# KinWaiCheuk/ReconVAT

Measured on AMD Instinct MI355X. Metric: training audio-sec/sec (node), higher is better.
Workload: dtype f32; 1 GPU; ReconVAT UNet_Onset VAT=True reconstruction=True, per-GPU B_l=8 + B_ul=8 segments of 327680 samples (640 frames x 229 mel), Adam+StepLR, fp32; parallelism=dp1, hipgraph=True, two_stream_schedule=True, kernel_plan_table=644fe159bb9eb70e, kernel_plan_mode=table, vat_nan_flag=0

## Files before the change

### reconvat_amd/csrc/attn.hip

```cpp
#include "common.h"
#include <stdlib.h>
#include <mutex>

#ifndef RV_ATTN_ABL
#define RV_ATTN_ABL 0
#endif
#define AT_W 31
#define AT_P 15
#define AT_TT 16
#define AT_WIN (AT_TT + 2 * AT_P)
#define AT_WINP 48
#define AT_NW 5
#define AT_NTHR (AT_NW * 64)
#define AT_SLD 80
#define AT_A2LD 52
#define AT_A3LD 84
#define AT_MAXT 4

struct AttnArgs {
    const float* q; const float* k; const float* v; long ld;
    const float* rel;
    float* out; float* att;
    const float* dout; const float* de_in;
    float* dq; float* dk; float* dv; long dld;
    float* de;
    int B, L, G, dh, dhp;
    int v4, dv4;
    int seq_kv;
    int rel_regs;
};

__device__ __attribute__((aligned(16))) const float rv_attn_zero[256] = {0.f};

__device__ __forceinline__ int stage_rows(float* dst, int ldk, const float* src, long ld, int col0, int dh, int dhp,
                                          int row0, int nvalid, int ntotal, int L, bool v4) {
    int issued = 0;
    const int wave = __builtin_amdgcn_readfirstlane(threadIdx.x >> 6), lane = threadIdx.x & 63;
    const int per = v4 ? 256 : 64;
    const int nfull = v4 ? (dh & ~3) : dh;
    const int ninst = (nfull + per - 1) / per;
    const int rem = dh - nfull;
    const int lf = v4 ? lane * 4 : lane;
    const float* s = src + ((long)(row0 + wave) * ld + col0) + lf;
    const float* z = rv_attn_zero + lf;
    float* drow = dst + wave * ldk;
    const long sstep = (long)AT_NW * ld;
    const int dstep = AT_NW * ldk;
    const int npad = dhp - dh;
    for (int r = wave; r < ntotal; r += AT_NW, s += sstep, drow += dstep) {
        const int t = row0 + r;
        const bool real = r < nvalid && t >= 0 && t < L;
        if (v4) {
            for (int k = 0; k < ninst; ++k)
                if (k * 256 + lf < nfull) glds16(real ? s + k * 256 : z, drow + k * 256);
            if (rem) {
                if (lane < rem) glds4(real ? s - lf + nfull + lane : rv_attn_zero + lane, drow + nfull);
                ++issued;
            }
        } else {
            for (int k = 0; k < ninst; ++k)
                if (k * 64 + lf < dh) glds4(real ? s + k * 64 : z, drow + k * 64);
        }
        issued += ninst;
        if (lane < npad) drow[dh + lane] = 0.f;
    }
    return issued;
}
__device__ __forceinline__ void stage_wait() { asm volatile("s_waitcnt vmcnt(0)" ::: "memory"); }

__device__ __forceinline__ f32x4 score_tile(const float* X, const float* Y, int ldk, int nchunk, int i, int g4) {
    f32x4 acc = (f32x4){0.f, 0.f, 0.f, 0.f};
    const float* xp = X + i * ldk + 4 * g4;
    const float* yp = Y + i * ldk + 4 * g4;
    for (int c = 0; c < nchunk; ++c) {
        const f32x4 a4 = *reinterpret_cast<const f32x4*>(xp + 16 * c);
        const f32x4 b4 = *reinterpret_cast<const f32x4*>(yp + 16 * c);
#pragma unroll
        for (int r = 0; r < 4; ++r) acc = __builtin_amdgcn_mfma_f32_16x16x4f32(a4[r], b4[r], acc, 0, 0, 0);
    }
    return acc;
}

__device__ __forceinline__ f32x4 score_tile_regs(const float* X, const f32x4 (&yb)[16], int ldk, int nchunk, int i, int g4) {
    f32x4 acc = (f32x4){0.f, 0.f, 0.f, 0.f};
    const float* xp = X + i * ldk + 4 * g4;
#pragma unroll
    for (int c = 0; c < 16; ++c) {
        if (c < nchunk) {
            const f32x4 a4 = *reinterpret_cast<const f32x4*>(xp + 16 * c);
#pragma unroll
            for (int r = 0; r < 4; ++r) acc = __builtin_amdgcn_mfma_f32_16x16x4f32(a4[r], yb[c][r], acc, 0, 0, 0);
        }
    }
    return acc;
}

struct RelFrag { f32x4 y[AT_MAXT][2]; };
__device__ __forceinline__ void rel_frag_load(RelFrag& rf, const float* relT, int F, int col0, int dh, int ntiles) {
    const int lane = threadIdx.x & 63, wave = threadIdx.x >> 6;
    const int i = lane & 15, g4 = lane >> 4;
#pragma unroll
    for (int q = 0; q < AT_MAXT; ++q) {
        const int f = 16 * (wave + AT_NW * q) + i;
        const bool fok = wave + AT_NW * q < ntiles && f < dh;
#pragma unroll
        for (int c = 0; c < 2; ++c)
#pragma unroll
            for (int r = 0; r < 4; ++r) {
                const int w = 16 * c + 4 * g4 + r;
                rf.y[q][c][r] = (fok && w < AT_W) ? relT[(long)w * F + col0 + f] : 0.f;
            }
    }
}

template <int NCH>
__device__ __forceinline__ void apply_tiles(const float* A, int lda, const float* Y, int ldk, int ntiles, float* dst,
                                            long dld, int col0, int dh, int nrows_valid, const RelFrag* rf = nullptr) {
    const int lane = threadIdx.x & 63, wave = threadIdx.x >> 6;
    const int i = lane & 15, g4 = lane >> 4;
    f32x4 acc[AT_MAXT];
#pragma unroll
    for (int q = 0; q < AT_MAXT; ++q) acc[q] = (f32x4){0.f, 0.f, 0.f, 0.f};
    if (rf) {
#pragma unroll
        for (int c = 0; c < 2; ++c) {
            const f32x4 a4 = *reinterpret_cast<const f32x4*>(A + i * lda + 16 * (NCH + c) + 4 * g4);
#pragma unroll
            for (int q = 0; q < AT_MAXT; ++q) {
                if (wave + AT_NW * q < ntiles) {
#pragma unroll
                    for (int r = 0; r < 4; ++r) acc[q] = __builtin_amdgcn_mfma_f32_16x16x4f32(a4[r], rf->y[q][c][r], acc[q], 0, 0, 0);
                }
            }
        }
    }
#pragma unroll
    for (int c = 0; c < NCH; ++c) {
        const f32x4 a4 = *reinterpret_cast<const f32x4*>(A + i * lda + 16 * c + 4 * g4);
        const float* yk = Y + (16 * c + 4 * g4) * ldk + i;
#pragma unroll
        for (int q = 0; q < AT_MAXT; ++q) {
            const int nt = wave + AT_NW * q;
            if (nt < ntiles) {
#pragma unroll
                for (int r = 0; r < 4; ++r)
                    acc[q] = __builtin_amdgcn_mfma_f32_16x16x4f32(a4[r], yk[r * ldk + 16 * nt], acc[q], 0, 0, 0);
            }
        }
    }
#pragma unroll
    for (int q = 0; q < AT_MAXT; ++q) {
        const int nt = wave + AT_NW * q;
        const int f = 16 * nt + i;
        if (nt >= ntiles || f >= dh) continue;
#pragma unroll
        for (int r = 0; r < 4; ++r) {
            const int t = 4 * g4 + r;
            if (t < nrows_valid) dst[(long)t * dld + col0 + f] = acc[q][r];
        }
    }
}

__device__ __forceinline__ float grp16_sum(float v) {
#pragma unroll
    for (int o = 8; o > 0; o >>= 1) v += __shfl_xor(v, o, 64);
    return v;
}
__device__ __forceinline__ float grp16_max(float v) {
#pragma unroll
    for (int o = 8; o > 0; o >>= 1) v = fmaxf(v, __shfl_xor(v, o, 64));
    return v;
}

__global__ __launch_bounds__(AT_NTHR) void attn_fwd_k(AttnArgs a) {
    extern __shared__ __attribute__((aligned(16))) float smem[];
    const int dh = a.dh, dhp = a.dhp, ldk = dhp + 4, nchunk = dhp >> 4, F = a.G * dh;
    float* Qs = smem;
    float* Kx = Qs + AT_TT * ldk;
    float* Sr = Kx + (a.rel_regs ? AT_WINP : 80) * ldk;
    float* A2 = Sr + AT_TT * AT_SLD;
    const int ntile = (a.L + AT_TT - 1) / AT_TT;
    const int bx = xcd_remap(blockIdx.x, gridDim.x);
    const int b = bx / ntile, t0 = (bx - b * ntile) * AT_TT;
    const int g = blockIdx.y;
    const int tid = threadIdx.x, lane = tid & 63, wave = tid >> 6;
    const int i = lane & 15, g4 = lane >> 4;
    const long boff = (long)b * a.L * a.ld;
    if (RV_ATTN_ABL & 16) return;
    if (!(RV_ATTN_ABL & 1)) {
    stage_rows(Qs, ldk, a.q + boff, a.ld, g * dh, dh, dhp, t0, AT_TT, AT_TT, a.L, a.v4);
    stage_rows(Kx, ldk, a.k + boff, a.ld, g * dh, dh, dhp, t0 - AT_P, AT_WIN, AT_WINP, a.L, a.v4);
    }
    f32x4 yb[16];
    if (a.rel_regs) {
        if (wave >= 3) {
            const int w = 16 * (wave - 3) + i;
            const float* rp = a.rel + (long)min(w, AT_W - 1) * F + g * dh + 4 * g4;
#pragma unroll
            for (int c = 0; c < 16; ++c)
#pragma unroll
                for (int r = 0; r < 4; ++r) yb[c][r] = (c < nchunk && w < AT_W && 16 * c + 4 * g4 + r < dh) ? rp[16 * c + r] : 0.f;
        }
    } else if (!(RV_ATTN_ABL & 1)) {
        stage_rows(Kx + AT_WINP * ldk, ldk, a.rel, F, g * dh, dh, dhp, 0, AT_W, 32, AT_W, a.dv4);
    }
    for (int idx = tid; idx < AT_TT * AT_A2LD; idx += AT_NTHR) A2[idx] = 0.f;
    stage_wait();
    __syncthreads();
    if (!(RV_ATTN_ABL & 2)) {
        const f32x4 s = (a.rel_regs && wave >= 3) ? score_tile_regs(Qs, yb, ldk, nchunk, i, g4)
                                                  : score_tile(Qs, Kx + 16 * wave * ldk, ldk, nchunk, i, g4);
#pragma unroll
        for (int r = 0; r < 4; ++r) Sr[(4 * g4 + r) * AT_SLD + 16 * wave + i] = s[r];
    }
    __syncthreads();
    if (!(RV_ATTN_ABL & 1)) stage_rows(Kx, ldk, a.v + boff, a.ld, g * dh, dh, dhp, t0 - AT_P, AT_WIN, AT_WINP, a.L, a.v4);
    if (tid < 256 && !(RV_ATTN_ABL & 4)) {
        const int t = tid >> 4, l = tid & 15;
        const float* sr = Sr + t * AT_SLD;
        const float e0 = sr[t + l] + sr[AT_WINP + l];
        const float e1 = l < 15 ? sr[t + l + 16] + sr[AT_WINP + l + 16] : -INFINITY;
        const float m = grp16_max(fmaxf(e0, e1));
        float p0 = expf(e0 - m), p1 = l < 15 ? expf(e1 - m) : 0.f;
        const float inv = 1.f / grp16_sum(p0 + p1);
        p0 *= inv; p1 *= inv;
        A2[t * AT_A2LD + t + l] = p0;
        if (l < 15) A2[t * AT_A2LD + t + l + 16] = p1;
        if (a.att && t0 + t < a.L) {
            float* ar = a.att + (((long)b * a.L + t0 + t) * a.G + g) * AT_W;
            ar[l] = p0;
            if (l < 15) ar[l + 16] = p1;
        }
    }
    stage_wait();
    __syncthreads();
    if (!(RV_ATTN_ABL & 8)) apply_tiles<3>(A2, AT_A2LD, Kx, ldk, nchunk, a.out + ((long)b * a.L + t0) * F, F, g * dh, dh, a.L - t0);
}

__global__ __launch_bounds__(AT_NTHR) void attn_bwd_q_k(AttnArgs a) {
    extern __shared__ __attribute__((aligned(16))) float smem[];
    const int dh = a.dh, dhp = a.dhp, ldk = dhp + 4, nchunk = dhp >> 4, F = a.G * dh;
    float* Ds = smem;
    float* Kx = Ds + AT_TT * ldk;
    float* Sr = Kx + (a.rel_regs ? AT_WINP : 80) * ldk;
    float* A3 = Sr + AT_TT * AT_SLD;
    const int ntile = (a.L + AT_TT - 1) / AT_TT;
    const int bx = xcd_remap(blockIdx.x, gridDim.x);
    const int b = bx / ntile, t0 = (bx - b * ntile) * AT_TT;
    const int g = blockIdx.y;
    const int tid = threadIdx.x, lane = tid & 63, wave = tid >> 6;
    const int i = lane & 15, g4 = lane >> 4;
    const long boff = (long)b * a.L * a.ld;
    stage_rows(Ds, ldk, a.dout + (long)b * a.L * F, F, g * dh, dh, dhp, t0, AT_TT, AT_TT, a.L, a.dv4);
    stage_rows(Kx, ldk, a.v + boff, a.ld, g * dh, dh, dhp, t0 - AT_P, AT_WIN, AT_WINP, a.L, a.v4);
    RelFrag rf;
    if (a.rel_regs) rel_frag_load(rf, a.rel, F, g * dh, dh, nchunk);
    else stage_rows(Kx + AT_WINP * ldk, ldk, a.rel, F, g * dh, dh, dhp, 0, AT_W, 32, AT_W, a.dv4);
    for (int idx = tid; idx < AT_TT * AT_A3LD; idx += AT_NTHR) A3[idx] = 0.f;
    stage_wait();
    __syncthreads();
    if (wave < 3) {
        const f32x4 s = score_tile(Ds, Kx + 16 * wave * ldk, ldk, nchunk, i, g4);
#pragma unroll
        for (int r = 0; r < 4; ++r) Sr[(4 * g4 + r) * AT_SLD + 16 * wave + i] = s[r];
    }
    __syncthreads();
    stage_rows(Kx, ldk, a.k + boff, a.ld, g * dh, dh, dhp, t0 - AT_P, AT_WIN, AT_WINP, a.L, a.v4);
    if (tid < 256) {
        const int t = tid >> 4, l = tid & 15;
        const bool rv = t0 + t < a.L;
        const long arow = (((long)b * a.L + t0 + t) * a.G + g) * AT_W;
        const float p0 = rv ? a.att[arow + l] : 0.f;
        const float p1 = (rv && l < 15) ? a.att[arow + l + 16] : 0.f;
        const float* sr = Sr + t * AT_SLD;
        const float d0 = sr[t + l], d1 = l < 15 ? sr[t + l + 16] : 0.f;
        const float dot = grp16_sum(p0 * d0 + p1 * d1);
        const float e0 = p0 * (d0 - dot), e1 = p1 * (d1 - dot);
        float* ar = A3 + t * AT_A3LD;
        ar[t + l] = e0;
        ar[AT_WINP + l] = e0;
        if (l < 15) { ar[t + l + 16] = e1; ar[AT_WINP + l + 16] = e1; }
        if (rv) {
            a.de[arow + l] = e0;
            if (l < 15) a.de[arow + l + 16] = e1;
        }
    }
    stage_wait();
    __syncthreads();
    if (a.rel_regs) apply_tiles<3>(A3, AT_A3LD, Kx, ldk, nchunk, a.dq + ((long)b * a.L + t0) * a.dld, a.dld, g * dh, dh, a.L - t0, &rf);
    else apply_tiles<5>(A3, AT_A3LD, Kx, ldk, nchunk, a.dq + ((long)b * a.L + t0) * a.dld, a.dld, g * dh, dh, a.L - t0);
}

__global__ __launch_bounds__(AT_NTHR) void attn_bwd_kv_k(AttnArgs a) {
    extern __shared__ __attribute__((aligned(16))) float smem[];
    const int dh = a.dh, dhp = a.dhp, ldk = dhp + 4, nchunk = dhp >> 4, F = a.G * dh;
    float* Yd = smem;
    float* Yq = a.seq_kv ? Yd : Yd + AT_WINP * ldk;
    float* Ca = Yq + AT_WINP * ldk;
    float* Ce = Ca + AT_WINP * 32;
    float* A4 = Ce + AT_WINP * 32;
    float* A5 = A4 + AT_TT * AT_A2LD;
    const int ntile = (a.L + AT_TT - 1) / AT_TT;
    const int bx = xcd_remap(blockIdx.x, gridDim.x);
    const int b = bx / ntile, s0 = (bx - b * ntile) * AT_TT;
    const int g = blockIdx.y;
    const int tid = threadIdx.x;
    stage_rows(Yd, ldk, a.dout + (long)b * a.L * F, F, g * dh, dh, dhp, s0 - AT_P, AT_WIN, AT_WINP, a.L, a.dv4);
    if (!a.seq_kv) stage_rows(Yq, ldk, a.q + (long)b * a.L * a.ld, a.ld, g * dh, dh, dhp, s0 - AT_P, AT_WIN, AT_WINP, a.L, a.v4);
    const long cld = (long)a.G * AT_W;
    stage_rows(Ca, 32, a.att + (long)b * a.L * cld, cld, g * AT_W, AT_W, 32, s0 - AT_P, AT_WIN, AT_WINP, a.L, false);
    stage_rows(Ce, 32, a.de_in + (long)b * a.L * cld, cld, g * AT_W, AT_W, 32, s0 - AT_P, AT_WIN, AT_WINP, a.L, false);
    stage_wait();
    __syncthreads();
    for (int idx = tid; idx < AT_TT * AT_A2LD; idx += AT_NTHR) {
        const int sl = idx / AT_A2LD, u = idx - sl * AT_A2LD;
        const int w = sl - u + 2 * AT_P;
        const bool in = u < AT_WIN && w >= 0 && w < AT_W;
        A4[idx] = in ? Ca[u * 32 + w] : 0.f;
        A5[idx] = in ? Ce[u * 32 + w] : 0.f;
    }
    __syncthreads();
    const long orow = ((long)b * a.L + s0) * a.dld;
    apply_tiles<3>(A4, AT_A2LD, Yd, ldk, nchunk, a.dv + orow, a.dld, g * dh, dh, a.L - s0);
    if (a.seq_kv) {
        __syncthreads();
        stage_rows(Yq, ldk, a.q + (long)b * a.L * a.ld, a.ld, g * dh, dh, dhp, s0 - AT_P, AT_WIN, AT_WINP, a.L, a.v4);
        stage_wait();
        __syncthreads();
    }
    apply_tiles<3>(A5, AT_A2LD, Yq, ldk, nchunk, a.dk + orow, a.dld, g * dh, dh, a.L - s0);
}

static bool attn_v4(int dh, long ld, const void* p) {
    static const int aligned_only = getenv("RV_ATTN_V4_ALIGNED") ? atoi(getenv("RV_ATTN_V4_ALIGNED")) : 0;
    if (!aligned_only) return true;
    return (dh % 4) == 0 && (ld % 4) == 0 && (((uintptr_t)p) & 15) == 0;
}

static int attn_setup(AttnArgs& a, int dh, const char* who) {
    RV_CHECK_ARG(dh >= 1 && dh <= 256, "%s: head dim %d unsupported", who, dh);
    a.dh = dh;
    a.dhp = (dh + 15) & ~15;
    static std::once_flag attr_once;
    std::call_once(attr_once, [] {
        (void)hipFuncSetAttribute((const void*)attn_fwd_k, hipFuncAttributeMaxDynamicSharedMemorySize, 128 * 1024);
        (void)hipFuncSetAttribute((const void*)attn_bwd_q_k, hipFuncAttributeMaxDynamicSharedMemorySize, 128 * 1024);
        (void)hipFuncSetAttribute((const void*)attn_bwd_kv_k, hipFuncAttributeMaxDynamicSharedMemorySize, 128 * 1024);
    });
    return RV_OK;
}

extern "C" {

int rv_local_attn_fwd(const float* q, const float* k, const float* v, long ld, const float* relT, float* out, float* att, int B,
                      int L, int G, int dh, void* stream) {
    AttnArgs a = {};
    const int rc = attn_setup(a, dh, "rv_local_attn_fwd");
    if (rc != RV_OK) return rc;
    RV_CHECK_ARG(ld >= (long)G * dh, "rv_local_attn_fwd: row stride %ld < G*dh", ld);
    a.q = q; a.k = k; a.v = v; a.ld = ld; a.rel = relT; a.out = out; a.att = att; a.B = B; a.L = L; a.G = G;
    a.v4 = attn_v4(dh, ld, q) && attn_v4(dh, ld, k) && attn_v4(dh, ld, v);
    a.dv4 = attn_v4(dh, (long)G * dh, relT);
    const int ntile = (L + AT_TT - 1) / AT_TT, ldk = a.dhp + 4;
    size_t lds = ((size_t)(AT_TT + 80) * ldk + AT_TT * AT_SLD + AT_TT * AT_A2LD) * sizeof(float);
    static const int relregs_env = getenv("RV_ATTN_REL_REGS") ? atoi(getenv("RV_ATTN_REL_REGS")) : 1;
    static const size_t occ_kb = getenv("RV_ATTN_OCC_KB") ? (size_t)atoi(getenv("RV_ATTN_OCC_KB")) : 78;
    a.rel_regs = relregs_env && lds > occ_kb * 1024;
    if (a.rel_regs) lds -= (size_t)32 * ldk * sizeof(float);
    hipLaunchKernelGGL(attn_fwd_k, dim3(B * ntile, G), dim3(AT_NTHR), lds, (hipStream_t)stream, a);
    RV_LAUNCH_CHECK("rv_local_attn_fwd");
    return RV_OK;
}

int rv_local_attn_bwd(const float* dout, const float* q, const float* k, const float* v, long ld, const float* relT,
                      const float* att, float* dq, float* dk, float* dv, long dld, float* de, int B, int L, int G, int dh,
                      void* stream) {
    hipStream_t st = (hipStream_t)stream;
    AttnArgs a = {};
    const int rc = attn_setup(a, dh, "rv_local_attn_bwd");
    if (rc != RV_OK) return rc;
    RV_CHECK_ARG(ld >= (long)G * dh && dld >= (long)G * dh, "rv_local_attn_bwd: row stride < G*dh");
    a.q = q; a.k = k; a.v = v; a.ld = ld; a.rel = relT; a.att = (float*)att; a.dout = dout;
    a.dq = dq; a.dk = dk; a.dv = dv; a.dld = dld; a.de = de; a.de_in = de; a.B = B; a.L = L; a.G = G;
    a.v4 = attn_v4(dh, ld, q) && attn_v4(dh, ld, k) && attn_v4(dh, ld, v);
    a.dv4 = attn_v4(dh, (long)G * dh, relT) && attn_v4(dh, (long)G * dh, dout);
    const int ntile = (L + AT_TT - 1) / AT_TT, ldk = a.dhp + 4;
    size_t lds1 = ((size_t)(AT_TT + 80) * ldk + AT_TT * AT_SLD + AT_TT * AT_A3LD) * sizeof(float);
    static const int relregs_env = getenv("RV_ATTN_REL_REGS") ? atoi(getenv("RV_ATTN_REL_REGS")) : 1;
    static const size_t occ_kb = getenv("RV_ATTN_OCC_KB") ? (size_t)atoi(getenv("RV_ATTN_OCC_KB")) : 78;
    a.rel_regs = relregs_env && lds1 > occ_kb * 1024;
    if (a.rel_regs) lds1 -= (size_t)32 * ldk * sizeof(float);
    hipLaunchKernelGGL(attn_bwd_q_k, dim3(B * ntile, G), dim3(AT_NTHR), lds1, st, a);
    RV_LAUNCH_CHECK("rv_local_attn_bwd(q)");
    const size_t lds_two = ((size_t)2 * AT_WINP * ldk + 2 * AT_WINP * 32 + 2 * AT_TT * AT_A2LD) * sizeof(float);
    a.seq_kv = lds_two > occ_kb * 1024;
    const size_t lds2 = lds_two - (a.seq_kv ? (size_t)AT_WINP * ldk * sizeof(float) : 0);
    hipLaunchKernelGGL(attn_bwd_kv_k, dim3(B * ntile, G), dim3(AT_NTHR), lds2, st, a);
    RV_LAUNCH_CHECK("rv_local_attn_bwd(kv)");
    return RV_OK;
}

}
```

Measured before the change: 16160 audio-s/s.

## Add 32-row local attention kernels with buffer-to-LDS staging and wave variants

Adds forward and backward local-attention kernels that handle 32 query rows per block instead of 16, so the 46-row key/value window overlaps less and halo loads are amortised over more rows. Staging now uses buffer loads that write straight into LDS, with out-of-range offsets handling padding and zero fill. The new path can run with 5 or 10 waves. It is the default unless an environment variable selects tile 16 or the tensors are too large for 32-bit buffer offsets. The trade-off is more LDS per block, which can lower occupancy, and fewer blocks in the grid.

```diff
diff --git a/reconvat_amd/csrc/attn.hip b/reconvat_amd/csrc/attn.hip
--- a/reconvat_amd/csrc/attn.hip
+++ b/reconvat_amd/csrc/attn.hip
@@ -1,4 +1,4 @@
-#include "common.h"
+#include "conv_shared.h"
 #include <stdlib.h>
 #include <mutex>
 
@@ -28,6 +28,8 @@
     int v4, dv4;
     int seq_kv;
     int rel_regs;
+    unsigned qkv_bytes, do_bytes, rel_bytes, co_bytes;
+    int rel_first;
 };
 
 __device__ __attribute__((aligned(16))) const float rv_attn_zero[256] = {0.f};
@@ -95,14 +97,16 @@
     return acc;
 }
 
-struct RelFrag { f32x4 y[AT_MAXT][2]; };
-__device__ __forceinline__ void rel_frag_load(RelFrag& rf, const float* relT, int F, int col0, int dh, int ntiles) {
+template <int MAXT> struct RelFragT { f32x4 y[MAXT][2]; };
+typedef RelFragT<AT_MAXT> RelFrag;
+template <int NW, int MAXT>
+__device__ __forceinline__ void rel_frag_load(RelFragT<MAXT>& rf, const float* relT, int F, int col0, int dh, int ntiles) {
     const int lane = threadIdx.x & 63, wave = threadIdx.x >> 6;
     const int i = lane & 15, g4 = lane >> 4;
 #pragma unroll
-    for (int q = 0; q < AT_MAXT; ++q) {
-        const int f = 16 * (wave + AT_NW * q) + i;
-        const bool fok = wave + AT_NW * q < ntiles && f < dh;
+    for (int q = 0; q < MAXT; ++q) {
+        const int f = 16 * (wave + NW * q) + i;
+        const bool fok = wave + NW * q < ntiles && f < dh;
 #pragma unroll
         for (int c = 0; c < 2; ++c)
 #pragma unroll
@@ -254,7 +258,7 @@
     stage_rows(Ds, ldk, a.dout + (long)b * a.L * F, F, g * dh, dh, dhp, t0, AT_TT, AT_TT, a.L, a.dv4);
     stage_rows(Kx, ldk, a.v + boff, a.ld, g * dh, dh, dhp, t0 - AT_P, AT_WIN, AT_WINP, a.L, a.v4);
     RelFrag rf;
-    if (a.rel_regs) rel_frag_load(rf, a.rel, F, g * dh, dh, nchunk);
+    if (a.rel_regs) rel_frag_load<AT_NW>(rf, a.rel, F, g * dh, dh, nchunk);
     else stage_rows(Kx + AT_WINP * ldk, ldk, a.rel, F, g * dh, dh, dhp, 0, AT_W, 32, AT_W, a.dv4);
     for (int idx = tid; idx < AT_TT * AT_A3LD; idx += AT_NTHR) A3[idx] = 0.f;
     stage_wait();
@@ -331,6 +335,325 @@
     apply_tiles<3>(A5, AT_A2LD, Yq, ldk, nchunk, a.dk + orow, a.dld, g * dh, dh, a.L - s0);
 }
 
+#define AT2_TT 32
+#define AT2_WIN (AT2_TT + 2 * AT_P)
+#define AT2_WINP 64
+#define AT2_SLD 96
+#define AT2_A2LD 68
+#define AT2_A3LD 100
+#define AT2_NSCORE 10
+
+#if defined(__HIP_DEVICE_COMPILE__)
+__device__ __forceinline__ void rv_buf_lds4(rv_rsrc_t rs, void* lds, unsigned voff) {
+    __builtin_amdgcn_raw_ptr_buffer_load_lds(rs, (__attribute__((address_space(3))) void*)lds, 4, voff, 0, 0, 0);
+}
+#else
+__device__ inline void rv_buf_lds4(rv_rsrc_t, void*, unsigned) {}
+#endif
+
+template <int NW>
+__device__ __forceinline__ void stage_rows_buf(float* dst, int ldk, const float* base, unsigned bytes, int ld, int dh, int dhp, int row0,
+                                               int nvalid, int ntotal, bool v4) {
+    const rv_rsrc_t rs = rv_make_rsrc(base, bytes);
+    const int wave = __builtin_amdgcn_readfirstlane(threadIdx.x >> 6), lane = threadIdx.x & 63;
+    const unsigned kColOut = 0x80000000u, kRowOut = 0x40000000u;
+    float* drow = dst + wave * ldk;
+    int rb = (row0 + wave) * ld * 4;
+    const int rstep = NW * ld * 4, dstep = NW * ldk;
+    if (v4) {
+        const int nfull = dh & ~3, rem = dh - nfull, zlo = nfull + (rem ? 4 : 0), lf = 4 * lane;
+        const bool act = lf < nfull || (lf >= zlo && lf < dhp);
+        const unsigned vo = lf < nfull ? lf * 4u : kColOut;
+        const unsigned vt = lane < rem ? (nfull + lane) * 4u : kColOut;
+        for (int r = wave; r < ntotal; r += NW, rb += rstep, drow += dstep) {
+            const unsigned ro = r < nvalid ? (unsigned)rb : kRowOut;
+            if (act) rv_buf_lds16(rs, drow, vo + ro);
+            if (rem && lane < 4) rv_buf_lds4(rs, drow + nfull, vt + ro);
+        }
+    } else {
+        for (int r = wave; r < ntotal; r += NW, rb += rstep, drow += dstep) {
+            const unsigned ro = r < nvalid ? (unsigned)rb : kRowOut;
+            for (int k = 0; k * 64 < dhp; ++k) {
+                const int f = k * 64 + lane;
+                if (f < dhp) rv_buf_lds4(rs, drow + k * 64, (f < dh ? f * 4u : kColOut) + ro);
+            }
+        }
+    }
+}
+
+__device__ __forceinline__ void win_tile32(int id, int& rt, int& ct) { rt = id >= 3; ct = id - 2 * rt; }
+
+template <int NW, bool REL>
+__device__ __forceinline__ void apply32(const float* A, int lda, const float* Y, int ldk, int ntiles, float* dst, long dld, int col0, int dh,
+                                        int nrows_valid, const float* Yrel = nullptr, const RelFragT<(16 + NW - 1) / NW>* rf = nullptr,
+                                        bool rel_first = false) {
+    constexpr int MAXT = (16 + NW - 1) / NW;
+    const int lane = threadIdx.x & 63, wave = threadIdx.x >> 6;
+    const int i = lane & 15, g4 = lane >> 4;
+    f32x4 acc[2][MAXT];
+#pragma unroll
+    for (int q = 0; q < MAXT; ++q) acc[0][q] = acc[1][q] = (f32x4){0.f, 0.f, 0.f, 0.f};
+    auto rel_part = [&]() {
+#pragma unroll
+        for (int c = 0; c < 2; ++c) {
+            const f32x4 a0 = *reinterpret_cast<const f32x4*>(A + i * lda + AT2_WINP + 16 * c + 4 * g4);
+            const f32x4 a1 = *reinterpret_cast<const f32x4*>(A + (16 + i) * lda + AT2_WINP + 16 * c + 4 * g4);
+#pragma unroll
+            for (int q = 0; q < MAXT; ++q) {
+                const int nt = wave + NW * q;
+                if (nt < ntiles) {
+                    f32x4 y;
+                    if (rf) y = rf->y[q][c];
+                    else {
+                        const float* yk = Yrel + (16 * c + 4 * g4) * ldk + 16 * nt + i;
+#pragma unroll
+                        for (int r = 0; r < 4; ++r) y[r] = yk[r * ldk];
+                    }
+#pragma unroll
+                    for (int r = 0; r < 4; ++r) acc[0][q] = __builtin_amdgcn_mfma_f32_16x16x4f32(a0[r], y[r], acc[0][q], 0, 0, 0);
+#pragma unroll
+                    for (int r = 0; r < 4; ++r) acc[1][q] = __builtin_amdgcn_mfma_f32_16x16x4f32(a1[r], y[r], acc[1][q], 0, 0, 0);
+                }
+            }
+        }
+    };
+    if (REL && rel_first) rel_part();
+#pragma unroll
+    for (int c = 0; c < 4; ++c) {
+        f32x4 a0 = (f32x4){0.f, 0.f, 0.f, 0.f}, a1 = a0;
+        if (c < 3) a0 = *reinterpret_cast<const f32x4*>(A + i * lda + 16 * c + 4 * g4);
+        if (c > 0) a1 = *reinterpret_cast<const f32x4*>(A + (16 + i) * lda + 16 * c + 4 * g4);
+        const float* yk = Y + (16 * c + 4 * g4) * ldk + i;
+#pragma unroll
+        for (int q = 0; q < MAXT; ++q) {
+            const int nt = wave + NW * q;
+            if (nt < ntiles) {
+                f32x4 y;
+#pragma unroll
+                for (int r = 0; r < 4; ++r) y[r] = yk[r * ldk + 16 * nt];
+                if (c < 3) {
+#pragma unroll
+                    for (int r = 0; r < 4; ++r) acc[0][q] = __builtin_amdgcn_mfma_f32_16x16x4f32(a0[r], y[r], acc[0][q], 0, 0, 0);
+                }
+                if (c > 0) {
+#pragma unroll
+                    for (int r = 0; r < 4; ++r) acc[1][q] = __builtin_amdgcn_mfma_f32_16x16x4f32(a1[r], y[r], acc[1][q], 0, 0, 0);
+                }
+            }
+        }
+    }
+    if (REL && !rel_first) rel_part();
+#pragma unroll
+    for (int q = 0; q < MAXT; ++q) {
+        const int nt = wave + NW * q;
+        const int f = 16 * nt + i;
+        if (nt >= ntiles || f >= dh) continue;
+#pragma unroll
+        for (int rt = 0; rt < 2; ++rt)
+#pragma unroll
+            for (int r = 0; r < 4; ++r) {
+                const int t = 16 * rt + 4 * g4 + r;
+                if (t < nrows_valid) dst[(long)t * dld + col0 + f] = acc[rt][q][r];
+            }
+    }
+}
+
+template <int NW>
+__global__ __launch_bounds__(NW * 64) void attn_fwd32_k(AttnArgs a) {
+    extern __shared__ __attribute__((aligned(16))) float smem[];
+    static_assert(AT2_NSCORE % NW == 0, "the score tiles divide over the waves");
+    constexpr int NTHR = NW * 64, TPW = AT2_NSCORE / NW;
+    const int dh = a.dh, dhp = a.dhp, ldk = dhp + 4, nchunk = dhp >> 4, F = a.G * dh;
+    float* Qs = smem;
+    float* Kx = Qs + AT2_TT * ldk;
+    float* Rx = Kx + AT2_WINP * ldk;
+    float* Sr = Rx + (a.rel_regs ? 0 : 32) * ldk;
+    float* A2 = Sr + AT2_TT * AT2_SLD;
+    const int ntile = (a.L + AT2_TT - 1) / AT2_TT;
+    const int bx = xcd_remap(blockIdx.x, gridDim.x);
+    const int b = bx / ntile, t0 = (bx - b * ntile) * AT2_TT;
+    const int g = blockIdx.y;
+    const int tid = threadIdx.x, lane = tid & 63, wave = __builtin_amdgcn_readfirstlane(tid >> 6);
+    const int i = lane & 15, g4 = lane >> 4;
+    const long boff = (long)b * a.L * a.ld + g * dh;
+    const int id0 = wave * TPW;
+    if (RV_ATTN_ABL & 16) return;
+    if (!(RV_ATTN_ABL & 1)) {
+        stage_rows_buf<NW>(Qs, ldk, a.q + boff, a.qkv_bytes, (int)a.ld, dh, dhp, t0, AT2_TT, AT2_TT, a.v4);
+        stage_rows_buf<NW>(Kx, ldk, a.k + boff, a.qkv_bytes, (int)a.ld, dh, dhp, t0 - AT_P, AT2_WIN, AT2_WINP, a.v4);
+    }
+    f32x4 yb[16];
+    if (a.rel_regs) {
+        if (id0 >= 6) {
+            const int w = 16 * ((id0 - 6) >> 1) + i;
+            const float* rp = a.rel + (long)min(w, AT_W - 1) * F + g * dh + 4 * g4;
+#pragma unroll
+            for (int c = 0; c < 16; ++c)
+#pragma unroll
+                for (int r = 0; r < 4; ++r) yb[c][r] = (c < nchunk && w < AT_W && 16 * c + 4 * g4 + r < dh) ? rp[16 * c + r] : 0.f;
+        }
+    } else if (!(RV_ATTN_ABL & 1)) {
+        stage_rows_buf<NW>(Rx, ldk, a.rel + g * dh, a.rel_bytes, F, dh, dhp, 0, AT_W, 32, a.dv4);
+    }
+    for (int idx = tid; idx < AT2_TT * AT2_A2LD; idx += NTHR) A2[idx] = 0.f;
+    stage_wait();
+    __syncthreads();
+    if (!(RV_ATTN_ABL & 2)) {
+#pragma unroll
+        for (int j = 0; j < TPW; ++j) {
+            const int id = id0 + j;
+            int rt, col;
+            f32x4 s;
+            if (id < 6) {
+                int ct;
+                win_tile32(id, rt, ct);
+                s = score_tile(Qs + 16 * rt * ldk, Kx + 16 * ct * ldk, ldk, nchunk, i, g4);
+                col = 16 * ct;
+            } else {
+                rt = (id - 6) & 1;
+                const int c = (id - 6) >> 1;
+                s = a.rel_regs ? score_tile_regs(Qs + 16 * rt * ldk, yb, ldk, nchunk, i, g4)
+                               : score_tile(Qs + 16 * rt * ldk, Rx + 16 * c * ldk, ldk, nchunk, i, g4);
+                col = AT2_WINP + 16 * c;
+            }
+#pragma unroll
+            for (int r = 0; r < 4; ++r) Sr[(16 * rt + 4 * g4 + r) * AT2_SLD + col + i] = s[r];
+        }
+    }
+    __syncthreads();
+    if (!(RV_ATTN_ABL & 1)) stage_rows_buf<NW>(Kx, ldk, a.v + boff, a.qkv_bytes, (int)a.ld, dh, dhp, t0 - AT_P, AT2_WIN, AT2_WINP, a.v4);
+    if (!(RV_ATTN_ABL & 4)) {
+        for (int t = tid >> 4; t < AT2_TT; t += NTHR / 16) {
+            const int l = tid & 15;
+            const float* sr = Sr + t * AT2_SLD;
+            const float e0 = sr[t + l] + sr[AT2_WINP + l];
+            const float e1 = l < 15 ? sr[t + l + 16] + sr[AT2_WINP + l + 16] : -INFINITY;
+            const float m = grp16_max(fmaxf(e0, e1));
+            float p0 = expf(e0 - m), p1 = l < 15 ? expf(e1 - m) : 0.f;
+            const float inv = 1.f / grp16_sum(p0 + p1);
+            p0 *= inv; p1 *= inv;
+            A2[t * AT2_A2LD + t + l] = p0;
+            if (l < 15) A2[t * AT2_A2LD + t + l + 16] = p1;
+            if (a.att && t0 + t < a.L) {
+                float* ar = a.att + (((long)b * a.L + t0 + t) * a.G + g) * AT_W;
+                ar[l] = p0;
+                if (l < 15) ar[l + 16] = p1;
+            }
+        }
+    }
+    stage_wait();
+    __syncthreads();
+    if (!(RV_ATTN_ABL & 8)) apply32<NW, false>(A2, AT2_A2LD, Kx, ldk, nchunk, a.out + ((long)b * a.L + t0) * F, F, g * dh, dh, a.L - t0);
+}
+
+template <int NW>
+__global__ __launch_bounds__(NW * 64) void attn_bwd_q32_k(AttnArgs a) {
+    extern __shared__ __attribute__((aligned(16))) float smem[];
+    constexpr int NTHR = NW * 64, TPW = AT2_NSCORE / NW, MAXT = (16 + NW - 1) / NW;
+    const int dh = a.dh, dhp = a.dhp, ldk = dhp + 4, nchunk = dhp >> 4, F = a.G * dh;
+    float* Ds = smem;
+    float* Kx = Ds + AT2_TT * ldk;
+    float* Rx = Kx + AT2_WINP * ldk;
+    float* Sr = Rx + (a.rel_regs ? 0 : 32) * ldk;
+    float* A3 = Sr + AT2_TT * AT2_SLD;
+    const int ntile = (a.L + AT2_TT - 1) / AT2_TT;
+    const int bx = xcd_remap(blockIdx.x, gridDim.x);
+    const int b = bx / ntile, t0 = (bx - b * ntile) * AT2_TT;
+    const int g = blockIdx.y;
+    const int tid = threadIdx.x, lane = tid & 63, wave = __builtin_amdgcn_readfirstlane(tid >> 6);
+    const int i = lane & 15, g4 = lane >> 4;
+    const long boff = (long)b * a.L * a.ld + g * dh;
+    stage_rows_buf<NW>(Ds, ldk, a.dout + (long)b * a.L * F + g * dh, a.do_bytes, F, dh, dhp, t0, AT2_TT, AT2_TT, a.dv4);
+    stage_rows_buf<NW>(Kx, ldk, a.v + boff, a.qkv_bytes, (int)a.ld, dh, dhp, t0 - AT_P, AT2_WIN, AT2_WINP, a.v4);
+    RelFragT<MAXT> rf;
+    if (a.rel_regs) rel_frag_load<NW>(rf, a.rel, F, g * dh, dh, nchunk);
+    else stage_rows_buf<NW>(Rx, ldk, a.rel + g * dh, a.rel_bytes, F, dh, dhp, 0, AT_W, 32, a.dv4);
+    for (int idx = tid; idx < AT2_TT * AT2_A3LD; idx += NTHR) A3[idx] = 0.f;
+    stage_wait();
+    __syncthreads();
+#pragma unroll
+    for (int j = 0; j < TPW; ++j) {
+        const int id = wave * TPW + j;
+        if (id < 6) {
+            int rt, ct;
+            win_tile32(id, rt, ct);
+            const f32x4 s = score_tile(Ds + 16 * rt * ldk, Kx + 16 * ct * ldk, ldk, nchunk, i, g4);
+#pragma unroll
+            for (int r = 0; r < 4; ++r) Sr[(16 * rt + 4 * g4 + r) * AT2_SLD + 16 * ct + i] = s[r];
+        }
+    }
+    __syncthreads();
+    stage_rows_buf<NW>(Kx, ldk, a.k + boff, a.qkv_bytes, (int)a.ld, dh, dhp, t0 - AT_P, AT2_WIN, AT2_WINP, a.v4);
+    for (int t = tid >> 4; t < AT2_TT; t += NTHR / 16) {
+        const int l = tid & 15;
+        const bool rv = t0 + t < a.L;
+        const long arow = (((long)b * a.L + t0 + t) * a.G + g) * AT_W;
+        const float p0 = rv ? a.att[arow + l] : 0.f;
+        const float p1 = (rv && l < 15) ? a.att[arow + l + 16] : 0.f;
+        const float* sr = Sr + t * AT2_SLD;
+        const float d0 = sr[t + l], d1 = l < 15 ? sr[t + l + 16] : 0.f;
+        const float dot = grp16_sum(p0 * d0 + p1 * d1);
+        const float e0 = p0 * (d0 - dot), e1 = p1 * (d1 - dot);
+        float* ar = A3 + t * AT2_A3LD;
+        ar[t + l] = e0;
+        ar[AT2_WINP + l] = e0;
+        if (l < 15) { ar[t + l + 16] = e1; ar[AT2_WINP + l + 16] = e1; }
+        if (rv) {
+            a.de[arow + l] = e0;
+            if (l < 15) a.de[arow + l + 16] = e1;
+        }
+    }
+    stage_wait();
+    __syncthreads();
+    float* dq = a.dq + ((long)b * a.L + t0) * a.dld;
+    if (a.rel_regs) apply32<NW, true>(A3, AT2_A3LD, Kx, ldk, nchunk, dq, a.dld, g * dh, dh, a.L - t0, nullptr, &rf, a.rel_first != 0);
+    else apply32<NW, true>(A3, AT2_A3LD, Kx, ldk, nchunk, dq, a.dld, g * dh, dh, a.L - t0, Rx, nullptr, a.rel_first != 0);
+}
+
+template <int NW>
+__global__ __launch_bounds__(NW * 64) void attn_bwd_kv32_k(AttnArgs a) {
+    extern __shared__ __attribute__((aligned(16))) float smem[];
+    constexpr int NTHR = NW * 64;
+    const int dh = a.dh, dhp = a.dhp, ldk = dhp + 4, nchunk = dhp >> 4, F = a.G * dh;
+    float* Yd = smem;
+    float* Yq = a.seq_kv ? Yd : Yd + AT2_WINP * ldk;
+    float* Ca = Yq + AT2_WINP * ldk;
+    float* Ce = Ca + AT2_WINP * 32;
+    float* A4 = Ce + AT2_WINP * 32;
+    float* A5 = A4 + AT2_TT * AT2_A2LD;
+    const int ntile = (a.L + AT2_TT - 1) / AT2_TT;
+    const int bx = xcd_remap(blockIdx.x, gridDim.x);
+    const int b = bx / ntile, s0 = (bx - b * ntile) * AT2_TT;
+    const int g = blockIdx.y;
+    const int tid = threadIdx.x;
+    const float* qb = a.q + (long)b * a.L * a.ld + g * dh;
+    stage_rows_buf<NW>(Yd, ldk, a.dout + (long)b * a.L * F + g * dh, a.do_bytes, F, dh, dhp, s0 - AT_P, AT2_WIN, AT2_WINP, a.dv4);
+    if (!a.seq_kv) stage_rows_buf<NW>(Yq, ldk, qb, a.qkv_bytes, (int)a.ld, dh, dhp, s0 - AT_P, AT2_WIN, AT2_WINP, a.v4);
+    const int cld = a.G * AT_W;
+    const long coff = (long)b * a.L * cld + g * AT_W;
+    stage_rows_buf<NW>(Ca, 32, a.att + coff, a.co_bytes, cld, AT_W, 32, s0 - AT_P, AT2_WIN, AT2_WINP, false);
+    stage_rows_buf<NW>(Ce, 32, a.de_in + coff, a.co_bytes, cld, AT_W, 32, s0 - AT_P, AT2_WIN, AT2_WINP, false);
+    stage_wait();
+    __syncthreads();
+    for (int idx = tid; idx < AT2_TT * AT2_A2LD; idx += NTHR) {
+        const int sl = idx / AT2_A2LD, u = idx - sl * AT2_A2LD;
+        const int w = sl - u + 2 * AT_P;
+        const bool in = u < AT2_WIN && w >= 0 && w < AT_W;
+        A4[idx] = in ? Ca[u * 32 + w] : 0.f;
+        A5[idx] = in ? Ce[u * 32 + w] : 0.f;
+    }
+    __syncthreads();
+    const long orow = ((long)b * a.L + s0) * a.dld;
+    apply32<NW, false>(A4, AT2_A2LD, Yd, ldk, nchunk, a.dv + orow, a.dld, g * dh, dh, a.L - s0);
+    if (a.seq_kv) {
+        __syncthreads();
+        stage_rows_buf<NW>(Yq, ldk, qb, a.qkv_bytes, (int)a.ld, dh, dhp, s0 - AT_P, AT2_WIN, AT2_WINP, a.v4);
+        stage_wait();
+        __syncthreads();
+    }
+    apply32<NW, false>(A5, AT2_A2LD, Yq, ldk, nchunk, a.dk + orow, a.dld, g * dh, dh, a.L - s0);
+}
+
 static bool attn_v4(int dh, long ld, const void* p) {
     static const int aligned_only = getenv("RV_ATTN_V4_ALIGNED") ? atoi(getenv("RV_ATTN_V4_ALIGNED")) : 0;
     if (!aligned_only) return true;
@@ -346,9 +669,32 @@
         (void)hipFuncSetAttribute((const void*)attn_fwd_k, hipFuncAttributeMaxDynamicSharedMemorySize, 128 * 1024);
         (void)hipFuncSetAttribute((const void*)attn_bwd_q_k, hipFuncAttributeMaxDynamicSharedMemorySize, 128 * 1024);
         (void)hipFuncSetAttribute((const void*)attn_bwd_kv_k, hipFuncAttributeMaxDynamicSharedMemorySize, 128 * 1024);
+        (void)hipFuncSetAttribute((const void*)attn_fwd32_k<5>, hipFuncAttributeMaxDynamicSharedMemorySize, 128 * 1024);
+        (void)hipFuncSetAttribute((const void*)attn_bwd_q32_k<5>, hipFuncAttributeMaxDynamicSharedMemorySize, 128 * 1024);
+        (void)hipFuncSetAttribute((const void*)attn_bwd_kv32_k<5>, hipFuncAttributeMaxDynamicSharedMemorySize, 128 * 1024);
+        (void)hipFuncSetAttribute((const void*)attn_fwd32_k<10>, hipFuncAttributeMaxDynamicSharedMemorySize, 128 * 1024);
+        (void)hipFuncSetAttribute((const void*)attn_bwd_q32_k<10>, hipFuncAttributeMaxDynamicSharedMemorySize, 128 * 1024);
+        (void)hipFuncSetAttribute((const void*)attn_bwd_kv32_k<10>, hipFuncAttributeMaxDynamicSharedMemorySize, 128 * 1024);
     });
     return RV_OK;
 }
+
+static int attn_env(const char* name) { return getenv(name) ? atoi(getenv(name)) : 0; }
+static const int g_attn_tile_env = attn_env("RV_ATTN_TILE"), g_attn_tile_wide_env = attn_env("RV_ATTN_TILE_WIDE");
+static const int g_attn_waves_env = attn_env("RV_ATTN_WAVES"), g_attn_waves_wide_env = attn_env("RV_ATTN_WAVES_WIDE");
+struct AttnForm { int tile, waves; };
+static AttnForm attn_form(int dh, int L, long max_ld) {
+    const bool wide = dh > 128;
+    const int tile = wide && g_attn_tile_wide_env ? g_attn_tile_wide_env : g_attn_tile_env;
+    const int waves = wide && g_attn_waves_wide_env ? g_attn_waves_wide_env : g_attn_waves_env;
+    AttnForm f;
+    f.tile = tile == 16 || tile == 32 ? tile : 32;
+    f.waves = waves == 5 || waves == 10 ? waves : 5;
+    if (((long)L + 64) * max_ld * 4 >= 0x3f000000L) f.tile = 16;
+    return f;
+}
+static unsigned attn_view_bytes(int L, long ld, int dh) { return (unsigned)((((long)L - 1) * ld + dh) * 4); }
+static const size_t kAttnMaxLds = 128 * 1024;
 
 extern "C" {
 
@@ -366,6 +712,19 @@
     static const int relregs_env = getenv("RV_ATTN_REL_REGS") ? atoi(getenv("RV_ATTN_REL_REGS")) : 1;
     static const size_t occ_kb = getenv("RV_ATTN_OCC_KB") ? (size_t)atoi(getenv("RV_ATTN_OCC_KB")) : 78;
     a.rel_regs = relregs_env && lds > occ_kb * 1024;
+    const AttnForm form = attn_form(dh, L, ld > (long)G * dh ? ld : (long)G * dh);
+    if (form.tile == 32) {
+        size_t lds32 = ((size_t)(AT2_TT + AT2_WINP + 32) * ldk + AT2_TT * AT2_SLD + AT2_TT * AT2_A2LD) * sizeof(float);
+        a.rel_regs = (relregs_env && lds32 > occ_kb * 1024) || lds32 > kAttnMaxLds;
+        if (a.rel_regs) lds32 -= (size_t)32 * ldk * sizeof(float);
+        a.qkv_bytes = attn_view_bytes(L, ld, dh);
+        a.rel_bytes = attn_view_bytes(AT_W, (long)G * dh, dh);
+        const dim3 grid(B * ((L + AT2_TT - 1) / AT2_TT), G);
+        if (form.waves == 10) hipLaunchKernelGGL((attn_fwd32_k<10>), grid, dim3(640), lds32, (hipStream_t)stream, a);
+        else hipLaunchKernelGGL((attn_fwd32_k<5>), grid, dim3(320), lds32, (hipStream_t)stream, a);
+        RV_LAUNCH_CHECK("rv_local_attn_fwd");
+        return RV_OK;
+    }
     if (a.rel_regs) lds -= (size_t)32 * ldk * sizeof(float);
     hipLaunchKernelGGL(attn_fwd_k, dim3(B * ntile, G), dim3(AT_NTHR), lds, (hipStream_t)stream, a);
     RV_LAUNCH_CHECK("rv_local_attn_fwd");
@@ -389,6 +748,30 @@
     static const int relregs_env = getenv("RV_ATTN_REL_REGS") ? atoi(getenv("RV_ATTN_REL_REGS")) : 1;
     static const size_t occ_kb = getenv("RV_ATTN_OCC_KB") ? (size_t)atoi(getenv("RV_ATTN_OCC_KB")) : 78;
     a.rel_regs = relregs_env && lds1 > occ_kb * 1024;
+    long max_ld = ld > (long)G * dh ? ld : (long)G * dh;
+    if (max_ld < (long)G * AT_W) max_ld = (long)G * AT_W;
+    const AttnForm form = attn_form(dh, L, max_ld);
+    if (form.tile == 32) {
+        a.rel_first = a.rel_regs;
+        size_t q32 = ((size_t)(AT2_TT + AT2_WINP + 32) * ldk + AT2_TT * AT2_SLD + AT2_TT * AT2_A3LD) * sizeof(float);
+        a.rel_regs = (relregs_env && q32 > occ_kb * 1024) || q32 > kAttnMaxLds;
+        if (a.rel_regs) q32 -= (size_t)32 * ldk * sizeof(float);
+        a.qkv_bytes = attn_view_bytes(L, ld, dh);
+        a.do_bytes = attn_view_bytes(L, (long)G * dh, dh);
+        a.rel_bytes = attn_view_bytes(AT_W, (long)G * dh, dh);
+        a.co_bytes = attn_view_bytes(L, (long)G * AT_W, AT_W);
+        const dim3 grid(B * ((L + AT2_TT - 1) / AT2_TT), G), block(form.waves * 64);
+        if (form.waves == 10) hipLaunchKernelGGL((attn_bwd_q32_k<10>), grid, block, q32, st, a);
+        else hipLaunchKernelGGL((attn_bwd_q32_k<5>), grid, block, q32, st, a);
+        RV_LAUNCH_CHECK("rv_local_attn_bwd(q)");
+        const size_t two32 = ((size_t)2 * AT2_WINP * ldk + 2 * AT2_WINP * 32 + 2 * AT2_TT * AT2_A2LD) * sizeof(float);
+        a.seq_kv = two32 > occ_kb * 1024;
+        const size_t kv32 = two32 - (a.seq_kv ? (size_t)AT2_WINP * ldk * sizeof(float) : 0);
+        if (form.waves == 10) hipLaunchKernelGGL((attn_bwd_kv32_k<10>), grid, block, kv32, st, a);
+        else hipLaunchKernelGGL((attn_bwd_kv32_k<5>), grid, block, kv32, st, a);
+        RV_LAUNCH_CHECK("rv_local_attn_bwd(kv)");
+        return RV_OK;
+    }
     if (a.rel_regs) lds1 -= (size_t)32 * ldk * sizeof(float);
     hipLaunchKernelGGL(attn_bwd_q_k, dim3(B * ntile, G), dim3(AT_NTHR), lds1, st, a);
     RV_LAUNCH_CHECK("rv_local_attn_bwd(q)");
```

Measured after the change: 16520 audio-s/s, median of 6. +2.3%, better.
